# IRVLUTD/GraspTrajOpt

Hardware: AMD Instinct MI355X
Metric: grasp trajectories/sec (higher is better)
Workload: dtype f64

## Files before the change

grasptrajopt_amd/csrc/gto_api.hip:

```cpp
#include <hip/hip_runtime.h>
#include <hipcub/hipcub.hpp>

#include <algorithm>
#include <atomic>
#include <climits>
#include <cmath>
#include <cstdio>
#include <cstdlib>
#include <cstring>
#include <string>
#include <chrono>
#include <memory>
#include <mutex>
#include <thread>
#include <utility>
#include <vector>

#include <sys/prctl.h>

#include "gto_kernels.h"
#include "gto_depth.h"
#include "gto_cloud.h"
#include "gto_retime.h"
#include "gto_observe.h"
// ... 3 lines not shown

#define GTO_VERSION GTO_ABI_VERSION
#ifndef GTO_OBS_DEEP_PD
#define GTO_OBS_DEEP_PD 8
#endif

static std::string g_create_error;

#define GTO_SWEEP_WGS 64

#define GTO_MAX_LANES 8
#define GTO_BASE_PIN_SLOTS 4
#define GTO_STAGE_SLOTS 8
#define GTO_NAP_US 50
#define GTO_NAP_FEW_US 10
#define GTO_OBS_DEEP_MAX 32

struct Tunables {
  int ahead = 8;
  int ahead_few = 4;
  int spec_rej = 4, spec_acc = 4, spec_deep = 32;
  int spec_rej_few = 2, spec_jobs = 20;
  int spec_streak = 4;
  int spec_acc_tail = 2, spec_streak_tail = 2, obs_tg_few_tail = 3;
  int spec_few = 64;
  int obs_deep = 1;
  int dbg_cut = 0;
  int dist_relax = 0;
  int obs_interleave = 2;
  int static_pos = 1;
  int pb_merge = 4;
  int prebroad = 1;
  int seed_pb = 1;
  double pb_min_gain = 0.10;
  int obs_tg = 3;
  int obs_tg_few = 2;
  int obs_tg_wide = 5;
  bool obs_tg_given = false;
  int few_instances = 192;
  int step_nw_few = 8;
  int slots = 512;
  int lanes_max = 1, lane_min = 256, adopt_below = 0;
  int item_hint_forced = 0;
  int item_grid = 1;
  bool debug_timing = false;
  bool lane_debug = false;
};

static void read_tunables(Tunables& t) {
  using F = int Tunables::*;
  struct Row { const char* name; F f, also1, also2; int lo, hi; };
  const int BIG = INT_MAX;
  static const Row rows[] = {
      {"GTO_AHEAD", &Tunables::ahead, &Tunables::ahead_few, nullptr, 1, BIG},
      {"GTO_SPEC_REJ", &Tunables::spec_rej, nullptr, nullptr, 1, GTO_KSPEC},
      {"GTO_SPEC_REJ_FEW", &Tunables::spec_rej_few, nullptr, nullptr, 1, GTO_KSPEC},
      {"GTO_SPEC_STREAK", &Tunables::spec_streak, &Tunables::spec_streak_tail, nullptr, 0, BIG},
      {"GTO_SPEC_STREAK_TAIL", &Tunables::spec_streak_tail, nullptr, nullptr, 0, BIG},
      {"GTO_SPEC_JOBS", &Tunables::spec_jobs, nullptr, nullptr, 1, BIG},
      {"GTO_SPEC_ACC", &Tunables::spec_acc, &Tunables::spec_acc_tail, nullptr, 1, GTO_KSPEC},
      {"GTO_SPEC_ACC_TAIL", &Tunables::spec_acc_tail, nullptr, nullptr, 1, GTO_KSPEC},
      {"GTO_SPEC_DEEP", &Tunables::spec_deep, nullptr, nullptr, 0, BIG},
      {"GTO_SPEC_FEW", &Tunables::spec_few, nullptr, nullptr, 0, BIG},
      {"GTO_OBS_DEEP", &Tunables::obs_deep, nullptr, nullptr, 0, 1},
      {"GTO_PREBROAD", &Tunables::prebroad, nullptr, nullptr, 0, 1},
      {"GTO_SEED_PB", &Tunables::seed_pb, nullptr, nullptr, 0, 1},
      {"GTO_PB_MERGE", &Tunables::pb_merge, nullptr, nullptr, 1, BIG},
      {"GTO_STATIC_POS", &Tunables::static_pos, nullptr, nullptr, 0, 1},
      {"GTO_OBS_INTERLEAVE", &Tunables::obs_interleave, nullptr, nullptr, 0, 2},
      {"GTO_DIST_RELAX", &Tunables::dist_relax, nullptr, nullptr, 0, 1},
      {"GTO_DEBUG_CUT", &Tunables::dbg_cut, nullptr, nullptr, INT_MIN, INT_MAX},
      {"GTO_ITEM_GRID", &Tunables::item_grid, nullptr, nullptr, 0, 1},
      {"GTO_ITEM_HINT", &Tunables::item_hint_forced, nullptr, nullptr, 0, BIG},
      {"GTO_SLOTS", &Tunables::slots, nullptr, nullptr, 1, BIG},
      {"GTO_LANES", &Tunables::lanes_max, nullptr, nullptr, 1, GTO_MAX_LANES},
      {"GTO_LANE_MIN", &Tunables::lane_min, nullptr, nullptr, 1, BIG},
      {"GTO_ADOPT", &Tunables::adopt_below, nullptr, nullptr, 0, BIG},
      {"GTO_OBS_TG", &Tunables::obs_tg, &Tunables::obs_tg_few, &Tunables::obs_tg_few_tail, 1, GTO_MAX_TG},
      {"GTO_OBS_TG_FEW", &Tunables::obs_tg_few, &Tunables::obs_tg_few_tail, nullptr, 1, GTO_MAX_TG},
      {"GTO_OBS_TG_FEW_TAIL", &Tunables::obs_tg_few_tail, nullptr, nullptr, 1, GTO_MAX_TG},
      {"GTO_OBS_TG_WIDE", &Tunables::obs_tg_wide, nullptr, nullptr, 1, GTO_MAX_TG},
      {"GTO_FEW_INSTANCES", &Tunables::few_instances, nullptr, nullptr, INT_MIN, INT_MAX},
  };
  for (const Row& r : rows) {
    const char* e = getenv(r.name);
    if (!e) continue;
    int v = atoi(e);
    v = r.lo == 0 && r.hi == 1 ? (v != 0) : std::max(r.lo, std::min(r.hi, v));
    for (F f : {r.f, r.also1, r.also2})
      if (f) t.*f = v;
  }
  t.obs_tg_given = getenv("GTO_OBS_TG") != nullptr;
  if (const char* e = getenv("GTO_STEP_NW_FEW")) t.step_nw_few = atoi(e) == 8 ? 8 : 4;
  if (const char* e = getenv("GTO_PB_MIN_GAIN")) t.pb_min_gain = atof(e);
  t.debug_timing = getenv("GTO_DEBUG_TIMING") != nullptr;
  t.lane_debug = getenv("GTO_LANE_DEBUG") != nullptr;
  if (t.dbg_cut) fprintf(stderr, "[gto] WARNING: GTO_DEBUG_CUT=%d cuts the obstacle kernel short: timing experiments only, RESULTS ARE GARBAGE\n", t.dbg_cut);
}

using DevBuf = Owned<hipFree>;
using PinBuf = Owned<hipHostFree>;

struct gto_handle {
  int device = 0;
  hipStream_t stream = nullptr;
  bool own_stream = true;
  std::string err;
  gto_solver_opts opts;
  RobotDev rb;
  DevBuf rb_buf, px_buf, py_buf, pz_buf, plink_buf, perm_buf, chunks_buf;
  RobotDev* d_rb = nullptr;
  double *d_px = nullptr, *d_py = nullptr, *d_pz = nullptr;
  int32_t *d_plink = nullptr, *d_perm = nullptr;
  Chunk* d_chunks = nullptr;
  std::vector<PbChunk> pbchunks;
  int pb_C = 0;
  DevBuf d_pbimg;
  std::vector<SceneDev> scenes;
  std::vector<std::vector<DevBuf>> scene_bufs;
  DevBuf scenes_buf;
  SceneDev* d_scenes = nullptr;
  DevBuf state, Qcur, Qtry, vis, screw, blocks, goalblk, ssfixed, ndone, qf, livebuf, qfs, wrecbuf, itembuf, seedmask;
  DevBuf counters;
  unsigned long long last_counters[4] = {0, 0, 0, 0};
  PinBuf h_ndone;
  PinBuf h_progress;
  unsigned long long* d_progress = nullptr;
  unsigned progress_tag = 0;
  Tunables tu;
  int spec_kmax = 1;
  DevBuf dbg;
  std::vector<DevBuf> spare;
  DevBuf in[GTO_STAGE_SLOTS], out[GTO_STAGE_SLOTS];
  PinBuf pin_in[GTO_STAGE_SLOTS], pin_out[GTO_STAGE_SLOTS];
  bool profiling = false;
  std::vector<hipEvent_t> ev;
  std::vector<int> ev_variant;
  std::vector<long long> ev_wgs;
  double last_ms = 0.0;
  int last_launches = 0;
  double prof_ms[GTO_PROF_VARIANTS] = {};
  long long prof_launches[GTO_PROF_VARIANTS] = {}, prof_wgs[GTO_PROF_VARIANTS] = {};
  unsigned long long prof_points[GTO_PROF_VARIANTS] = {};
  size_t lm_lds = 0;
  int np = GTO_NB;
  DevBuf zws;
  hipStream_t lane_stream[GTO_MAX_LANES] = {};
  hipEvent_t lane_event[GTO_MAX_LANES] = {};
  hipStream_t user_lane_stream[GTO_MAX_LANES] = {};
  int n_user_lane_streams = 0;
  double items_per_job_prior = 0.0;
  std::mutex* prof_mu = nullptr;
  DevBuf rt_fac, rt_S, rt_flag, rt_P1, rt_P2, rt_cap, rt_X, rt_T, rt_stat;
  bool rt_fac_ready = false;
  DevBuf ck_xyz, ck_flags, ck_base;
// ... 867 lines not shown
  sp.tol_step = o.tol_step;
  sp.tol_rel_f = o.tol_rel_f;
  sp.lambda0 = o.lambda0;
  sp.dbg_cut = h->tu.dbg_cut;
  sp.interleave = h->tu.obs_interleave == 1;
  sp.static_pos = 0;
  sp.pb_next = 0, sp.pb_tg = 1, sp.pb_ng = 1, sp.pb_pw = 1, sp.pb_verify = 0;
  sp.pb_C = h->pb_C, sp.pb_tab0 = 0, sp.pb_mC = ObsGeom::magic(std::max(1, h->pb_C)), sp.pb_mF = ObsGeom::magic(h->rb.n_frames);
  sp.pb_eps = h->rb.pb_eps;
  sp.pb_npar = h->rb.pb_npar;
  sp.round = sp.parity = 0;
  sp.kcap = h->np == GTO_NB ? GTO_KSPEC : 1;
  sp.k_acc = sp.k_rej = sp.k_eval = 1;
  sp.spec_streak = h->tu.spec_streak;
  return sp;
}

static int ensure_workspace(gto_handle* h, int B) {
  const RobotDev& rb = h->rb;
  const size_t T = h->opts.T, n = rb.n_opt;
  int rc;
  if ((rc = ensure(h, h->state, (size_t)B * sizeof(InstState)))) return rc;
  if ((rc = ensure(h, h->Qcur, (size_t)B * n * T * sizeof(double)))) return rc;
  const size_t kcap = h->np == GTO_NB ? GTO_KSPEC : 1;
  if ((rc = ensure(h, h->Qtry, kcap * B * n * T * sizeof(double)))) return rc;
  const size_t bstride = (size_t)h->np * h->np + h->np + 8;
  if ((rc = ensure(h, h->blocks, (kcap + 1) * B * T * bstride * sizeof(double)))) return rc;
  if ((rc = ensure(h, h->goalblk, (kcap + 1) * B * 2 * bstride * sizeof(double)))) return rc;
  if ((rc = ensure(h, h->ssfixed, (size_t)B * 4 * sizeof(double)))) return rc;
  if ((rc = ensure(h, h->ndone, 64 * GTO_MAX_LANES))) return rc;
  if ((rc = ensure(h, h->qf, (size_t)B * T * rb.n_frames * sizeof(double)))) return rc;
  if ((rc = ensure(h, h->wrecbuf, (size_t)(kcap + 1) * B * T * 8 * sizeof(double)))) return rc;
  if ((rc = ensure(h, h->seedmask, (size_t)B * sizeof(unsigned long long)))) return rc;
  if (!h->h_ndone) HIPCHK(h, pinned_alloc(h->h_ndone, 64));
  if (!h->h_progress) {
    HIPCHK(h, pinned_alloc(h->h_progress, 64 * GTO_MAX_LANES, hipHostMallocMapped));
    std::memset(h->h_progress.get(), 0, 64 * GTO_MAX_LANES);
    HIPCHK(h, hipHostGetDevicePointer((void**)&h->d_progress, h->h_progress.get(), 0));
  }
  return GTO_OK;
}

static BatchPtrs make_ptrs(gto_handle* h, const int32_t* scene_id, const double* qc, const double* goals,
                           const int32_t* n_goals, const double* standoff, const double* base_pos, const double* Q0) {
  BatchPtrs bp = {};
  bp.scene_id = scene_id;
  bp.qc = qc;
  bp.goals = goals;
  bp.n_goals = n_goals;
  bp.standoff = standoff;
  bp.base_pos = base_pos;
  bp.Q0 = Q0;
  bp.state = h->state.as<InstState>();
  bp.Qcur = h->Qcur.as<double>();
  bp.Qtry = h->Qtry.as<double>();
  bp.blocks = h->blocks.as<double>();
  bp.goalblk = h->goalblk.as<double>();
  bp.ss_fixed = h->ssfixed.as<double>();
  bp.n_done = h->ndone.as<int32_t>();
  bp.qf = h->qf.as<double>();
  bp.live = nullptr;
  bp.jobs = nullptr;
  bp.nlive = nullptr;
  bp.next = nullptr;
  bp.qfs = nullptr;
  bp.wrec = h->wrecbuf.as<double>();
// ... 17 lines not shown
    if ((e = hipEventCreate(&ev_)) == hipSuccess) h->ev.push_back(ev_);
  }
  if (e == hipSuccess) {
    if (h->ev_variant.size() <= (size_t)h->last_launches) h->ev_variant.resize(h->last_launches + 1), h->ev_wgs.resize(h->last_launches + 1);
    h->ev_variant[h->last_launches] = variant;
    h->ev_wgs[h->last_launches] = wgs;
    e = hipEventRecord(h->ev[2 * h->last_launches], st);
  }
  if (e != hipSuccess && h->prof_mu) h->prof_mu->unlock();
  HIPCHK(h, e);
  return GTO_OK;
}
static int prof_end(gto_handle* h, hipStream_t st) {
  const hipError_t e = hipEventRecord(h->ev[2 * h->last_launches + 1], st);
  h->last_launches++;
  if (h->prof_mu) h->prof_mu->unlock();
  HIPCHK(h, e);
  return GTO_OK;
}

using InitKernel = decltype(&k_lm_init<GTO_NB>);
static InitKernel lm_init_kernel(int np) { return np == GTO_NB ? k_lm_init<GTO_NB> : k_lm_init<16>; }

struct ObsLaunch {
  int t_begin = 2, nT = 0;
  int fixed_mode = 0;
  bool timed = false;
  bool goal_terms = false;
  int n_jobs = 0;
  int tg = 0;
  bool deep = false;
  bool itemized = false;
  int items_hint = 0;
};
static ObsLaunch init_pass() {
  ObsLaunch o;
  o.t_begin = 0, o.nT = 4, o.fixed_mode = 1;
  return o;
}

static int launch_obstacle(gto_handle* h, hipStream_t st, const BatchPtrs& bp, const SolveParams& sp, int B, const ObsLaunch& o) {
  const int TG = o.fixed_mode ? 1 : std::max(1, std::min(o.tg > 0 ? o.tg : h->tu.obs_tg, o.nT));
  const ObsGeom geo(h->rb.n_cframes, h->rb.n_frames, h->rb.fk_rounds_c, h->rb.n_links, h->rb.n_opt, h->rb.n_chunks, TG, o.nT, h->np);
  const int nG = geo.nG;
  const int nb = o.n_jobs > 0 ? o.n_jobs : B;
  int n_regular = obstacle_grid(nb, nG);
  const bool sweep = o.itemized && o.items_hint > 0 && o.items_hint + GTO_SWEEP_WGS < n_regular && bp.live != nullptr && !o.fixed_mode && !o.deep && h->np == GTO_NB;
  if (sweep) n_regular = 8 * ((o.items_hint + 7) / 8);
  const size_t lds = (size_t)geo.lay.total_doubles * sizeof(double);
  const int n_crew = sweep ? GTO_SWEEP_WGS : 0;
  const dim3 grid(n_regular + n_crew + (o.goal_terms ? 8 * ((nb + 31) / 32) : 0));
  const bool deep_v = h->np == GTO_NB && o.deep;
  if (o.timed) {
    int rc_ = prof_begin(h, st, deep_v ? GTO_PROF_OBSTACLE_FEW : GTO_PROF_OBSTACLE, (long long)grid.x);
    if (rc_) return rc_;
  }
  BatchPtrs bpl = bp;
  if (bpl.work) bpl.work += 64 * (deep_v ? GTO_PROF_OBSTACLE_FEW : GTO_PROF_OBSTACLE);
  const bool listed = bp.live != nullptr && !o.fixed_mode;
  const int32_t* jobs_par = listed ? bp.jobs + (size_t)sp.parity * bp.cap * sp.kcap : nullptr;
  const int32_t* njobs_par = listed ? bp.nlive + GTO_NJOBS(sp.parity) : nullptr;
  const size_t items_cap = (size_t)bp.cap * sp.kcap * (sp.T - 2) + GTO_ITEM_SLACK;
  const int2* items_par = listed && o.itemized ? bp.items + (size_t)sp.parity * items_cap : nullptr;
  const int32_t* nitems_par = listed && o.itemized ? bp.nlive + 8 + sp.parity : nullptr;
  const bool hot = !o.fixed_mode && sp.grad_mode == GTO_GRAD_CENTRAL_DIFF;
  hipLaunchKernelGGL(obstacle_kernel(h->np, o.deep, sweep, hot), grid, dim3(256), lds, st, jobs_par, njobs_par, items_par, nitems_par, geo.nG, geo.m_nG, n_regular, B,
                     h->d_rb, h->d_px, h->d_py, h->d_pz, h->d_chunks, h->d_scenes, bpl, sp, o.t_begin, o.nT, o.fixed_mode, geo, n_crew);
  if (o.timed) return prof_end(h, st);
  return GTO_OK;
}

}

struct LaneCtx {
  hipStream_t st = nullptr;
  BatchPtrs bp;
  SolveParams sp;
  int lo = 0, n = 0, W = 0, cap = 0;
  int room = 0;
  int span_prev = 0;
  int n_resp = 0;
  int k = 0, known_done = 0, seen_round = -1, k_prev = 1;
  int last_plain = -1;
  bool items_ready = false, pb_off = false, handed = false;
  double ratio_max = 0.0;
  long end_us = 0, few_us = 0;
  unsigned long long* h_prog = nullptr;
};

struct Handover { int lane, parity, count, k_prev; };

struct SolveCall {
  gto_handle* h = nullptr;
  int B = 0, L = 1, T = 0, kcap = 1, nF = 0, max_iter = 0;
  int pb_ng = 1;
  bool pb_able = false;
  size_t lane_zws[GTO_MAX_LANES + 1] = {0};
  LaneCtx lanes[GTO_MAX_LANES];
  std::chrono::steady_clock::time_point tp_start;
  std::mutex mu;
  std::vector<Handover> requests;
  int reserved = 0;
  int adopt_limit = 0;
  std::atomic<int> rem0_pub{0}, others_open{0}, failed{0};
};

static int setup_lanes(gto_handle* h, hipStream_t st, SolveParams& sp, BatchPtrs& bp, SolveCall& c) {
  const int B = c.B, T = c.T, kcap = c.kcap, nF = c.nF;
  const int L = c.L = std::max(1, std::min(std::min(h->tu.lanes_max, GTO_MAX_LANES), B / std::max(1, h->tu.lane_min)));
  const int adopt_room = L > 1 ? (L - 1) * std::max(0, h->tu.adopt_below) : 0;
  size_t off_live[GTO_MAX_LANES + 1] = {0}, off_qfs[GTO_MAX_LANES + 1] = {0}, off_items[GTO_MAX_LANES + 1] = {0};
  for (int l = 0; l < L; ++l) {
    LaneCtx& ln = c.lanes[l];
    ln.lo = (int)((long long)B * l / L);
    ln.n = (int)((long long)B * (l + 1) / L) - ln.lo;
    ln.W = std::min(ln.n, h->tu.slots);
    ln.cap = ln.W + (l == 0 ? adopt_room : 0);
// ... 30 lines not shown
    else if (l < h->n_user_lane_streams) ln.st = h->user_lane_stream[l];
    else {
      if (!h->lane_stream[l]) {
        int lo_p = 0, hi_p = 0;
        HIPCHK(h, hipDeviceGetStreamPriorityRange(&lo_p, &hi_p));
        HIPCHK(h, hipStreamCreateWithPriority(&h->lane_stream[l], hipStreamNonBlocking, hi_p));
      }
      ln.st = h->lane_stream[l];
    }
    if (!h->lane_event[l]) HIPCHK(h, hipEventCreateWithFlags(&h->lane_event[l], hipEventDisableTiming));
  }
  HIPCHK(h, hipMemsetAsync(h->ndone.get(), 0, 16 * sizeof(int32_t) * L, st));
  h->progress_tag = h->progress_tag + 1 ? h->progress_tag + 1 : 1;
  for (int l = 0; l < L; ++l) c.lanes[l].bp.progress_tag = (unsigned long long)h->progress_tag << 32;
  if (h->profiling) {
    if ((rc = ensure(h, h->counters, GTO_PROF_VARIANTS * 64 * sizeof(unsigned long long)))) return rc;
    HIPCHK(h, hipMemsetAsync(h->counters.get(), 0, GTO_PROF_VARIANTS * 64 * sizeof(unsigned long long), st));
    bp.work = h->counters.as<unsigned long long>();
    for (int l = 0; l < L; ++l) c.lanes[l].bp.work = bp.work;
  }
  const int pb_tg = std::max(1, std::min(h->tu.obs_tg, T - 2));
  c.pb_ng = (T - 2 + pb_tg - 1) / pb_tg;
  const PbLayout pbl(T, h->rb.n_frames, h->pb_C, h->rb.pb_npar);
  c.pb_able = h->tu.prebroad && h->np == GTO_NB && c.pb_ng <= 64 && h->tu.obs_interleave != 1 && h->rb.n_xst <= GTO_PB_PARK && pbl.pw >= 1 && h->pb_C >= 1;
  for (int l = 0; l < L; ++l) {
    SolveParams& lsp = c.lanes[l].sp;
    lsp.pb_tg = pb_tg, lsp.pb_ng = c.pb_ng, lsp.pb_pw = std::max(1, pbl.pw), lsp.pb_tab0 = pbl.tab0;
    lsp.pb_verify = h->tu.dbg_cut == 10;
  }
  sp.pb_tg = pb_tg, sp.pb_ng = c.pb_ng, sp.pb_pw = std::max(1, pbl.pw), sp.pb_tab0 = pbl.tab0;
  return GTO_OK;
}

static int test_waiting_seeds(gto_handle* h, hipStream_t st, SolveCall& c) {
  if (!c.pb_able || !h->tu.seed_pb) return GTO_OK;
  for (int l = 0; l < c.L; ++l) {
    LaneCtx& ln = c.lanes[l];
    if (ln.n <= ln.W || ln.W <= h->tu.few_instances) continue;
    int rc;
    if (h->profiling && (rc = prof_begin(h, st, GTO_PROF_SEED_TEST, ln.n - ln.W))) return rc;
    hipLaunchKernelGGL(k_seed_broad, dim3(ln.n - ln.W), dim3(256), h->lm_lds, st, h->d_rb, ln.bp, ln.sp, c.B, h->seedmask.as<unsigned long long>());
    if (h->profiling && (rc = prof_end(h, st))) return rc;
    ln.bp.seed_mask = h->seedmask.as<unsigned long long>();
  }
  return GTO_OK;
}

enum StepVariant { STEP_FULL, STEP_FEW, STEP_WIDE };
struct RoundPlan {
  int in_flight = 0;
  int span = 0;
  bool few = false;
  bool interleave = false;
  ObsLaunch obs;
  StepVariant step = STEP_FULL;
  int k_acc = 1, k_rej = 1, spec_streak = 0;
  bool pb_next = false, static_pos = false;
  int k_next = 1;
  bool pb_off = false;
  double ratio_max = 0.0;
};

static RoundPlan plan_round(const gto_handle* h, const SolveCall& c, const LaneCtx& ln) {
  const Tunables& tu = h->tu;
  RoundPlan p;
  p.in_flight = std::min(ln.room, ln.n_resp - ln.known_done);
  p.few = p.in_flight <= tu.few_instances;
  p.span = ln.span_prev ? ln.span_prev : p.in_flight;
  p.interleave = tu.obs_interleave == 1 || (tu.obs_interleave == 2 && p.few);
  p.pb_off = ln.pb_off;
  p.ratio_max = ln.ratio_max;
  p.k_next = ln.k_prev;
  const bool large_call = ln.n_resp > tu.spec_deep;
  ObsLaunch& o = p.obs;
  o.nT = c.T - 2;
  o.timed = h->profiling;
  o.goal_terms = true;
  o.n_jobs = p.span * ln.k_prev;
  o.tg = p.few ? (large_call ? tu.obs_tg_few_tail : tu.obs_tg_few) : tu.obs_tg;
  o.deep = p.few && tu.obs_deep && p.in_flight <= GTO_OBS_DEEP_MAX;
  o.itemized = ln.items_ready && !p.few;
  if (o.itemized && tu.item_grid) {
    const unsigned long long p2 = __atomic_load_n(ln.h_prog + 2, __ATOMIC_RELAXED);
    const int jobs_bound = p.in_flight * ln.k_prev;
    const bool zero_ok = ln.last_plain < ln.seen_round - 1;
    if ((unsigned)(p2 >> 32) == h->progress_tag && ((p2 & 0xfffffull) > 0 || zero_ok) && (p2 & 0xfffffull) < 0xfffffull) {
      const double items_seen = (double)(p2 & 0xfffffull), jobs_seen = (double)((p2 >> 20) & 0xfffull);
      o.items_hint = (int)(1.5 * items_seen) + 256;
      if (jobs_seen > 0 && jobs_seen < 4095) p.ratio_max = std::max(p.ratio_max, items_seen / jobs_seen);
    } else if (h->items_per_job_prior > 0.0) {
      o.items_hint = (int)(1.25 * h->items_per_job_prior * jobs_bound) + 256;
    }
    if (tu.item_hint_forced > 0) o.items_hint = tu.item_hint_forced;
  }
  if (h->np != GTO_NB) {
    p.step = STEP_WIDE;
  } else if (p.few && tu.step_nw_few == 8) {
    p.step = STEP_FEW;
    const int k_budget = std::max(1, tu.spec_jobs / std::max(1, p.in_flight));
    p.k_acc = p.in_flight <= std::min(tu.spec_deep, tu.spec_few) ? std::min(std::min(large_call ? tu.spec_acc_tail : tu.spec_acc, k_budget), h->spec_kmax) : 1;
    p.spec_streak = large_call ? tu.spec_streak_tail : tu.spec_streak;
    p.k_rej = p.in_flight <= tu.spec_few ? std::min(std::max(std::min(tu.spec_rej, k_budget), tu.spec_rej_few), h->spec_kmax) : 1;
    p.k_next = std::max(p.k_acc, p.k_rej);
  } else {
    p.step = STEP_FULL;
    const bool pb_ok = c.pb_able && std::min(ln.W, ln.n) > tu.few_instances;
    if (pb_ok && !p.pb_off && !ln.sp.pb_verify) {
      const unsigned long long p2 = __atomic_load_n(ln.h_prog + 2, __ATOMIC_RELAXED);
      if ((unsigned)(p2 >> 32) == h->progress_tag) {
        const double jobs_seen = (double)((p2 >> 20) & 0xfffull), items_seen = (double)(p2 & 0xfffffull);
        if (jobs_seen > 0 && items_seen > 0 && jobs_seen < 4095 && ln.k >= 12 && items_seen > (1.0 - tu.pb_min_gain) * jobs_seen * c.pb_ng) p.pb_off = true;
      }
    }
    p.pb_next = pb_ok && !p.pb_off && !p.few;
    p.static_pos = tu.static_pos && c.L == 1 && !p.few;
    p.k_next = 1;
  }
  return p;
}
// ... 274 lines not shown
  int n_in_ = 0, n_out_ = 0;
  void* host_[GTO_STAGE_SLOTS] = {};
  size_t bytes_[GTO_STAGE_SLOTS] = {};
};

extern "C" {

int gto_solve_batch_device(gto_handle* h, int32_t B, int32_t n_max, const int32_t* scene_id, const double* qc,
                           const double* goals, const int32_t* n_goals, const double* standoff, const double* base_pos,
                           const double* Q0, double* Q_out, double* dQ_out, double* cost_out, int32_t* iters_out,
                           int32_t* status_out, void* stream) {
  if (!h) return GTO_ERR_INVALID_ARG;
  if (B < 0 || n_max < 1) return fail(h, GTO_ERR_INVALID_ARG, "B must be >= 0 and n_max >= 1");
  if (B == 0) return GTO_OK;
  if (B > GTO_JOB_MASK) return fail(h, GTO_ERR_UNSUPPORTED, "more than 16.7 million instances in one call");
  if (!scene_id || !qc || !goals || !n_goals || !base_pos || !Q0) return fail(h, GTO_ERR_INVALID_ARG, "null input array");
  if (h->scenes.empty()) return fail(h, GTO_ERR_NO_SCENE, "no scene has been set");
  HIPCHK(h, hipSetDevice(h->device));
  hipStream_t st = stream ? (hipStream_t)stream : h->stream;
  int rc = ensure_workspace(h, B);
  if (rc) return rc;
  SolveParams sp = make_params(h, n_max, standoff != nullptr);
  BatchPtrs bp = make_ptrs(h, scene_id, qc, goals, n_goals, standoff, base_pos, Q0);
  h->last_launches = 0;
  h->last_ms = 0.0;
  if (h->dbg) HIPCHK(h, hipMemsetAsync(h->dbg.as<long long>() + 40, 0, 216 * sizeof(long long), st));

  SolveCall c;
  c.h = h, c.B = B, c.T = sp.T, c.kcap = sp.kcap, c.nF = h->rb.n_frames, c.max_iter = sp.max_iter;
  if ((rc = setup_lanes(h, st, sp, bp, c))) return rc;
  const int L = c.L;
  for (int l = 0; l < L; ++l)
    hipLaunchKernelGGL(lm_init_kernel(h->np), dim3(c.lanes[l].n), dim3(256), 0, st, h->d_rb, c.lanes[l].bp, c.lanes[l].sp, B, 0);
  if ((rc = launch_obstacle(h, st, bp, sp, B, init_pass()))) return rc;
  if ((rc = test_waiting_seeds(h, st, c))) return rc;
  if (L > 1) {
    HIPCHK(h, hipEventRecord(h->lane_event[0], st));
    for (int l = 0; l < L; ++l) HIPCHK(h, hipStreamWaitEvent(c.lanes[l].st, h->lane_event[0], 0));
  }
  const int old_slack = prctl(PR_GET_TIMERSLACK);
  if (old_slack > 1000) (void)prctl(PR_SET_TIMERSLACK, 1000UL);
  c.tp_start = std::chrono::steady_clock::now();
  int rc_loop = run_lanes(c);
  {
    double r_ = 0.0;
    for (int l = 0; l < L; ++l) r_ = std::max(r_, c.lanes[l].ratio_max);
    if (r_ > 0.0) h->items_per_job_prior = r_;
  }
  for (int l = 0; l < L && L > 1 && !rc_loop; ++l)
    if (!c.lanes[l].handed) {
      if (hipEventRecord(h->lane_event[l], c.lanes[l].st) != hipSuccess || hipStreamWaitEvent(st, h->lane_event[l], 0) != hipSuccess) {
        h->err = "solve loop: joining the lanes failed";
        rc_loop = GTO_ERR_HIP;
      }
    }
  if (rc_loop)
    for (int l = 0; l < L && L > 1; ++l) (void)hipStreamSynchronize(c.lanes[l].st);
  bp.live = c.lanes[0].bp.live, bp.cap = c.lanes[0].bp.cap;
  if (old_slack > 1000) (void)prctl(PR_SET_TIMERSLACK, (unsigned long)old_slack);
  if (rc_loop) return rc_loop;
  hipLaunchKernelGGL(k_lm_finalize, dim3(B), dim3(64), 0, st, h->d_rb, bp, sp, B, Q_out, dQ_out, cost_out, iters_out, status_out);
  HIPCHK(h, hipGetLastError());
  if (h->dbg && (rc = print_debug_stamps(h, st))) return rc;
  if (h->profiling && (rc = harvest_profile(h, st, bp.work))) return rc;
  return GTO_OK;
}

// ... 455 lines not shown
  int rc = check_scene_ids_host(h, scene_id, B);
  if (rc) return rc;
  HIPCHK(h, hipSetDevice(h->device));
  const size_t ndof = h->rb.ndof, T = h->opts.T;
  std::vector<double> dummy_goal;
  std::vector<int32_t> dummy_n;
  std::vector<double> qc(B * ndof);
  for (int b = 0; b < B; ++b)
    for (size_t i = 0; i < ndof; ++i) qc[b * ndof + i] = Q[((size_t)b * ndof + i) * T];
  if (!with_goals) {
    n_max = 1;
    dummy_goal.assign((size_t)B * 16, 0.0);
    for (int b = 0; b < B; ++b) dummy_goal[b * 16] = dummy_goal[b * 16 + 5] = dummy_goal[b * 16 + 10] = dummy_goal[b * 16 + 15] = 1.0;
    dummy_n.assign(B, 1);
    goals = dummy_goal.data();
    n_goals = dummy_n.data();
    standoff = nullptr;
  }
  Staging io(h);
  const int32_t *d_sid, *d_ng;
  const double *d_qc, *d_goals, *d_so, *d_base, *d_Q0;
  if ((rc = io.in(scene_id, B, &d_sid))) return rc;
  if ((rc = io.in(qc.data(), B * ndof, &d_qc))) return rc;
  if ((rc = io.in(goals, (size_t)B * n_max * 16, &d_goals))) return rc;
  if ((rc = io.in(n_goals, B, &d_ng))) return rc;
  if ((rc = io.in(standoff, (size_t)B * 16, &d_so))) return rc;
  if ((rc = io.in(base_pos, (size_t)B * 3, &d_base))) return rc;
  if ((rc = io.in(Q, B * ndof * T, &d_Q0))) return rc;
  if ((rc = ensure_workspace(h, B))) return rc;
  SolveParams sp = make_params(h, n_max, standoff != nullptr);
  BatchPtrs bp = make_ptrs(h, d_sid, d_qc, d_goals, d_ng, d_so, d_base, d_Q0);
  HIPCHK(h, hipMemsetAsync(bp.n_done, 0, sizeof(int32_t), h->stream));
  hipLaunchKernelGGL(lm_init_kernel(h->np), dim3(B), dim3(256), 0, h->stream, h->d_rb, bp, sp, B, 1 );
  if ((rc = launch_obstacle(h, h->stream, bp, sp, B, init_pass()))) return rc;
  h->last_launches = 0;
  ObsLaunch ev;
  ev.nT = (int)T - 2, ev.timed = h->profiling;
  if ((rc = launch_obstacle(h, h->stream, bp, sp, B, ev))) return rc;
  if (h->profiling) {
    HIPCHK(h, hipStreamSynchronize(h->stream));
    float ms = 0.f;
    HIPCHK(h, hipEventElapsedTime(&ms, h->ev[0], h->ev[1]));
    h->last_ms = ms;
  }
  states.resize(B);
  const size_t bstride = (size_t)h->np * h->np + h->np + 8;
  blocks.resize((size_t)B * T * bstride);
  ssfixed.resize((size_t)B * 4);
  HIPCHK(h, hipMemcpyAsync(states.data(), h->state.get(), B * sizeof(InstState), hipMemcpyDeviceToHost, h->stream));
  HIPCHK(h, hipMemcpyAsync(blocks.data(), h->blocks.as<double>() + (size_t)1 * B * T * bstride,
                           blocks.size() * sizeof(double), hipMemcpyDeviceToHost, h->stream));
  HIPCHK(h, hipMemcpyAsync(ssfixed.data(), h->ssfixed.get(), ssfixed.size() * sizeof(double), hipMemcpyDeviceToHost, h->stream));
  HIPCHK(h, hipStreamSynchronize(h->stream));
  HIPCHK(h, hipGetLastError());
  return GTO_OK;
}

int gto_eval_objective(gto_handle* h, int32_t B, int32_t n_max, const int32_t* scene_id, const double* goals,
                       const int32_t* n_goals, const double* standoff, const double* base_pos, const double* Q,
                       double* f_goal, double* f_obs, double* f_vel, int32_t* goal_argmin) {
  if (!h) return GTO_ERR_INVALID_ARG;
  if (B < 0 || n_max < 1 || !scene_id || !goals || !n_goals || !base_pos || !Q) return fail(h, GTO_ERR_INVALID_ARG, "bad argument");
  if (B == 0) return GTO_OK;
  std::vector<InstState> st;
  std::vector<double> blocks, ssf;
  int rc = eval_common(h, B, n_max, scene_id, goals, n_goals, standoff, base_pos, Q, true, st, blocks, ssf);
  if (rc) return rc;
// ... 1135 lines not shown
```

grasptrajopt_amd/csrc/gto_kernels.h:

```cpp
#pragma once
#include <type_traits>

#include "gto_device.h"

template <int NP>
struct Blk {
  static constexpr int JTJ = 0, JTR = NP * NP, SS = NP * NP + NP, STRIDE = NP * NP + NP + 8;
};
#define BLK_JTJ 0
#define BLK_JTR 64
#define BLK_SS 72
#define BLK_STRIDE 80
#define GTO_MAX_ACTIVE 256
#define GTO_MAX_TG 8
#define GTO_MAX_T 96
#ifndef GTO_LIST_CAP
#define GTO_LIST_CAP 64
#endif

#define GTO_KSPEC 4
#define GTO_JOB_SHIFT 28
#define GTO_JOB_SET_SHIFT 24
#define GTO_JOB_MASK 0x00ffffff
#define GTO_JOB_ENTRY(b, set, cand) ((b) | ((set) << GTO_JOB_SET_SHIFT) | ((cand) << GTO_JOB_SHIFT))
// ... 618 lines not shown
  const int par = sp.parity, NS = sp.kcap + 1;
  if (!SWEEP && listed && bid == 0 && tid == 0) {
    bp.nlive[GTO_NLIVE(1 - par)] = bp.nlive[GTO_NJOBS(1 - par)] = 0;
    bp.nlive[8 + 1 - par] = 0;
  }
  if (is_goal) {
    if (gi_ >= n_act || le < 0) return;
    const int bg = le & GTO_JOB_MASK, gcand = le >> GTO_JOB_SHIFT;
    if (bp.state[bg].done || (listed && bp.state[bg].first)) return;
    double* s_fr2 = smem_obs + wave * GTO_GOAL_SCRATCH(NP);
    double* s_q2 = s_fr2 + 2 * GTO_MAX_FRAMES * 12;
    double* s_ga = s_q2 + 2 * GTO_MAX_DOF;
    double* s_gs = s_ga + 48;
#ifdef GTO_DEBUG_LONGEST_WG
    const bool dbg_goal = bp.dbg && bg == 0 && gcand == 0 && lane == 0;
    if (dbg_goal) bp.dbg[31] = clock64();
#endif
    trial_goal_terms_wave<NP>(rb, bp, sp, B, bg, lane, listed ? GTO_JOB_SET(le) : (bp.state[bg].slot + 1 + gcand) % NS, gcand, bp.state + bg, s_q2, s_fr2, s_ga, s_gs);
#ifdef GTO_DEBUG_LONGEST_WG
    if (dbg_goal) bp.dbg[32] = clock64();
#endif
    return;
  }
  for (;;) {
  {
  const int t0v = t_begin + grp_id * TG;
  const bool static_only = fixed_mode && t0v >= 2;
  const int t0w = static_only ? 0 : t0v;
  const bool inter = sp.interleave && !fixed_mode;
  const int wstep = inter ? nG : 1, w0 = inter ? t_begin + grp_id : t0w;
  const int ng = static_only ? 1 : (inter ? geo.q_nT + (grp_id < geo.r_nT ? 1 : 0) : min(TG, (fixed_mode ? 2 : t_begin + nT) - t0v));
  auto wp = [&](int kq_) { return w0 + kq_ * wstep; };
  if (sp.dbg_cut == 5 && (le >= 0 || bi < 0)) goto next_item;

  const int bic = min(bi, (listed ? bp.cap * sp.kcap : B) - 1);
  const int Fq = geo.Fq;
  const double* __restrict__ qfp = listed ? bp.qfs + ((((size_t)par * bp.cap * sp.kcap + bic) * T) + w0) * Fq : bp.qf + ((size_t)bic * T + w0) * Fq;
  const int qstride = wstep * Fq;
  const int tq = fast_div(tid, F, geo.m_F);
  const int fo_t = tid < ng * F ? rb->cf_orig[tid - tq * F] : -1;
  const int jtv = tid < ng * F ? rb->cf_type[tid - tq * F] : GTO_JOINT_FIXED;
  const double qfv = fo_t >= 0 ? qfp[fo_t + tq * qstride] : 0.0;
  const int nt = geo.nt;
  double tabv[6];
#pragma unroll
  for (int u = 0; u < 6; ++u) tabv[u] = tid + 256 * u < nt ? rb->fk_tab_c[tid + 256 * u] : 0.0;
  if ((itemized ? rbid : bi) >= n_act || le < 0) goto next_item;
  const int b = le & GTO_JOB_MASK, cand = le >> GTO_JOB_SHIFT;
  const bool sparse = listed;
  const InstState* st = bp.state + b;
  const bool dbg_wg = bp.dbg && b == 0 && grp_id == nG - 1;
#ifdef GTO_DEBUG_LONGEST_WG
  const long long t_wg0 = bp.dbg ? clock64() : 0;
#endif
  if (dbg_wg && tid == 0) bp.dbg[10] = clock64();
  if (sp.dbg_cut == 6) goto next_item;
  if (!listed && st->done) goto next_item;
  const int set_out = listed ? GTO_JOB_SET(le) : (st->slot + 1 + cand) % NS;
  const int C = geo.C;
  double ssfix = 0.0;
  if (!fixed_mode && tid < ng) ssfix = bp.ss_fixed[4 * b + (wp(tid) < sp.ts ? 2 : 3)];
#pragma unroll
  for (int u = 0; u < 6; ++u)
    if (tid + 256 * u < nt) s_ktab[tid + 256 * u] = tabv[u];
  for (int k = tid + 256 * 6; k < nt; k += 256) s_ktab[k] = rb->fk_tab_c[k];
  if (sp.dbg_cut == 7) goto next_item;
// ... 1040 lines not shown
  const int* s_flag = reinterpret_cast<const int*>(s_tab);
  const double ss_a = s_tab[38], ss_o = s_tab[39];
  double* __restrict__ wr = bp.wrec + (((size_t)set_n * B + b) * T + 2) * 8;
  for (int i = tid; i < m * 8; i += NT) {
    const int sI = i >> 3;
    if (!s_flag[sI / TG]) wr[i] = (i & 7) == 0 ? 0.0 + (sI + 2 < sp.ts ? ss_a : ss_o) : 0.0;
  }
}
__device__ __forceinline__ void pb_list_groups(const BatchPtrs& bp, const SolveParams& sp, int par_n, int entry, int pos, bool hit, int lane) {
  const bool on = lane < sp.pb_ng && (hit || sp.pb_verify);
  const unsigned long long mask = __ballot(on);
  int base = 0;
  if (lane == 0 && mask) base = atomicAdd(bp.nlive + 8 + par_n, __popcll(mask));
  base = __shfl(base, 0, 64);
  if (on) bp.items[(size_t)par_n * ((size_t)bp.cap * sp.kcap * (sp.T - 2) + GTO_ITEM_SLACK) + base + __popcll(mask & ((1ull << lane) - 1ull))] =
              make_int2(entry, (pos << 8) | lane | (hit ? 0 : 0x80));
}

template <int NT>
__device__ __forceinline__ void prebroad_tail(const RobotDev* __restrict__ rb,
                                              const BatchPtrs& bp, const SolveParams& sp, int B, int b, int scene_b, int set_n, int pos_next,
                                              const double* __restrict__ s_qt, double* __restrict__ smem, int tid) {
  const bool dbg_t = bp.dbg && b == 0 && tid == 0;
  pb_test<NT>(rb, bp, sp, b, scene_b, s_qt, smem, tid, true);
  if (dbg_t) bp.dbg[38] = clock64();
  pb_settle_records<NT>(bp, sp, B, b, set_n, smem, tid);
  if (tid < 64) {
    const int* s_flag = reinterpret_cast<const int*>(smem + sp.pb_tab0);
    pb_list_groups(bp, sp, 1 - sp.parity, GTO_JOB_ENTRY(b, set_n, 0), pos_next, tid < sp.pb_ng && s_flag[tid] != 0, tid);
  }
  if (dbg_t) bp.dbg[39] = clock64();
}

__global__ __launch_bounds__(256) void k_seed_broad(const RobotDev* __restrict__ rb, BatchPtrs bp, SolveParams sp, int B, unsigned long long* __restrict__ mask_out) {
  constexpr int NT = 256;
  const int b = bp.b0 + bp.w0 + blockIdx.x, tid = threadIdx.x;
  if (b >= bp.n_total) return;
  extern __shared__ __attribute__((aligned(16))) double smem[];
  __shared__ int s_bad;
  const int T = sp.T, m = T - 2, n = rb->n_opt, F = rb->n_frames;
  double* __restrict__ s_qt = smem + 80 * (size_t)m;
  const int scene_b = bp.scene_id[b];
  if (tid == 0) s_bad = 0;
  __syncthreads();
  {
    const double* __restrict__ qf0 = bp.qf + (size_t)b * T * F;
    bool bad = false;
    for (int i = tid; i < T * F; i += NT) bad |= !(fabs(qf0[i]) < INFINITY);
    if (bad) s_bad = 1;
    const double* __restrict__ Qt = bp.Qtry + (size_t)b * n * T;
    for (int i = tid; i < m * 8; i += NT) s_qt[i] = (i & 7) < n ? Qt[(size_t)(i & 7) * T + (i >> 3) + 2] : 0.0;
  }
  __syncthreads();
  if (s_bad) {
    if (tid == 0) mask_out[b] = ~0ull;
    return;
  }
  pb_test<NT>(rb, bp, sp, b, scene_b, s_qt, smem, tid, false);
  pb_settle_records<NT>(bp, sp, B, b, 1, smem, tid);
  if (tid < 64) {
    const int* s_flag = reinterpret_cast<const int*>(smem + sp.pb_tab0);
    const unsigned long long mk = __ballot(tid < sp.pb_ng && s_flag[tid] != 0);
    if (tid == 0) mask_out[b] = mk;
  }
}

template <int NP>
__global__ __launch_bounds__(256) void k_lm_init(const RobotDev* __restrict__ rb, BatchPtrs bp, SolveParams sp, int B, int raw) {
  const int b = blockIdx.x + bp.b0, tid = threadIdx.x, bl = blockIdx.x;
  __shared__ double s_gaff[48];
  __shared__ double s_gscr[2 * NP * 6];
  __shared__ double s_q[2 * GTO_MAX_DOF];
  __shared__ double s_fr[2 * GTO_MAX_FRAMES * 12];
  const int T = sp.T, n = rb->n_opt;
  InstState* st = bp.state + b;
  if (tid == 0) {
    st->f = INFINITY;
    st->lambda = sp.lambda0;
    st->nu = 2.0;
    st->pred[0] = 0.0;
    st->ncand = 1;
    st->cflags = 0;
    st->nz0 = st->nz1 = 0ull;
    st->slot = 0;
    st->first = 1;
    st->done = 0;
    st->status = GTO_STATUS_MAX_ITER;
    st->evals = 0;
    st->argmin_cur = 0;
  }
  if (bp.live && tid == 0) {
    if (bl < bp.w0) bp.live[bl] = b, bp.jobs[bl] = GTO_JOB_ENTRY(b, 1, 0);
    if (bl == 0) {
      *bp.next = bp.b0 + bp.w0;
      bp.nlive[GTO_NLIVE(0)] = bp.nlive[GTO_NJOBS(0)] = bp.w0;
      bp.nlive[GTO_NLIVE(1)] = bp.nlive[GTO_NJOBS(1)] = 0;
      bp.nlive[8] = bp.nlive[9] = 0;
    }
  }
  const double* Q0b = bp.Q0 + (size_t)b * rb->ndof * T;
  double* Qt = bp.Qtry + (size_t)b * n * T;
  double* Qc = bp.Qcur + (size_t)b * n * T;
  for (int idx = tid; idx < n * T; idx += 256) {
    const int j = idx / T, t = idx % T;
    double v = Q0b[(size_t)rb->opt_index[j] * T + t];
    if (!raw) {
      if (t < 2) v = bp.qc[(size_t)b * rb->ndof + rb->opt_index[j]];
      else v = v < rb->lower[j] ? rb->lower[j] : (v > rb->upper[j] ? rb->upper[j] : v);
    }
    Qt[idx] = v;
    Qc[idx] = v;
  }
  __syncthreads();
  {
    const int F = rb->n_frames;
    double* qf = bp.qf + (size_t)b * T * F;
    for (int idx = tid; idx < T * F; idx += 256) {
      const int t = idx / F, i = idx - t * F, dq = rb->q_index[i];
      double v = 0.0;
      if (dq >= 0) {
        const int j = rb->opt_of_dof[dq];
        v = j >= 0 ? Qt[(size_t)j * T + t] : Q0b[(size_t)dq * T + t];
      }
      qf[idx] = v;
      if (bp.live && bl < bp.w0) bp.qfs[(size_t)bl * T * F + idx] = v;
    }
  }
  if (tid < 64) trial_goal_terms_wave<NP>(rb, bp, sp, B, b, tid, 1, 0, st, s_q, s_fr, s_gaff, s_gscr);
}

__device__ __forceinline__ double fast_rcp(double x) {
  double r = __builtin_amdgcn_rcp(x);
  r = fma(fma(-x, r, 1.0), r, r);
  r = fma(fma(-x, r, 1.0), r, r);
  return r;
}

template <int J>
__device__ __forceinline__ double bcast_col8(double v) {
  constexpr int q = J & 3, QP = q | (q << 2) | (q << 4) | (q << 6);
  constexpr int BM = (J >> 2) ? 0x5 : 0xA;
  int lo = __builtin_amdgcn_update_dpp(0, __double2loint(v), QP, 0xf, 0xf, false);
  int hi = __builtin_amdgcn_update_dpp(0, __double2hiint(v), QP, 0xf, 0xf, false);
  lo = __builtin_amdgcn_update_dpp(lo, lo, 0x141, 0xf, BM, false);
  hi = __builtin_amdgcn_update_dpp(hi, hi, 0x141, 0xf, BM, false);
  return __hiloint2double(hi, lo);
}
template <int J>
__device__ __forceinline__ void gj_pivot8(double& S, int& bad, int r, int c) {
  const double pjj = __hiloint2double(__builtin_amdgcn_readlane(__double2hiint(S), J * 9),
                                      __builtin_amdgcn_readlane(__double2loint(S), J * 9));
  const double prj = bcast_col8<J>(S);
  const double pjc = __shfl(S, J * 8 + c, 64);
  if (!(pjj > 0.0)) bad = 1;
  const double piv = fast_rcp(pjj);
  const double tcol = -prj * piv;
  const double in_row = (c == J) ? piv : pjc * piv;
  const double off_row = (c == J) ? tcol : fma(tcol, pjc, S);
  S = (r == J) ? in_row : off_row;
}
__device__ __forceinline__ int gj_invert8(double& S, int r, int c, int n = 8) {
// ... 2443 lines not shown
```

Measured before the change: 570,400.

## Deduplicate identical instances in init obstacle pass and seed-broadphase all slots

Adds a kernel that, within each 64-instance wave group, finds instances whose scene, base pose and first two timesteps of joint frames match their predecessor, and maps each to a representative head. The fixed-mode init obstacle pass skips non-head instances, and a spread kernel copies the head's fixed terms to the duplicates. It also runs the seed broadphase test on the in-slot instances so their group lists are prepared up front, and ignores progress hints from those seeded rounds. This avoids redundant collision work when batches contain repeated starts, at the cost of extra launches and reliance on exact bitwise equality.

```diff
diff --git a/grasptrajopt_amd/csrc/gto_api.hip b/grasptrajopt_amd/csrc/gto_api.hip
--- a/grasptrajopt_amd/csrc/gto_api.hip
+++ b/grasptrajopt_amd/csrc/gto_api.hip
@@ -59,6 +59,8 @@
   int pb_merge = 4;
   int prebroad = 1;
   int seed_pb = 1;
+  int seed_pb_all = 1;
+  int init_dedup = 1, init_dedup_min = 1280;
   double pb_min_gain = 0.10;
   int obs_tg = 3;
   int obs_tg_few = 2;
@@ -92,6 +94,9 @@
       {"GTO_OBS_DEEP", &Tunables::obs_deep, nullptr, nullptr, 0, 1},
       {"GTO_PREBROAD", &Tunables::prebroad, nullptr, nullptr, 0, 1},
       {"GTO_SEED_PB", &Tunables::seed_pb, nullptr, nullptr, 0, 1},
+      {"GTO_SEED_PB_ALL", &Tunables::seed_pb_all, nullptr, nullptr, 0, 1},
+      {"GTO_INIT_DEDUP", &Tunables::init_dedup, nullptr, nullptr, 0, 1},
+      {"GTO_INIT_DEDUP_MIN", &Tunables::init_dedup_min, nullptr, nullptr, 0, BIG},
       {"GTO_PB_MERGE", &Tunables::pb_merge, nullptr, nullptr, 1, BIG},
       {"GTO_STATIC_POS", &Tunables::static_pos, nullptr, nullptr, 0, 1},
       {"GTO_OBS_INTERLEAVE", &Tunables::obs_interleave, nullptr, nullptr, 0, 2},
@@ -147,7 +152,7 @@
   std::vector<std::vector<DevBuf>> scene_bufs;
   DevBuf scenes_buf;
   SceneDev* d_scenes = nullptr;
-  DevBuf state, Qcur, Qtry, vis, screw, blocks, goalblk, ssfixed, ndone, qf, livebuf, qfs, wrecbuf, itembuf, seedmask;
+  DevBuf state, Qcur, Qtry, vis, screw, blocks, goalblk, ssfixed, ndone, qf, livebuf, qfs, wrecbuf, itembuf, seedmask, inithead;
   DevBuf counters;
   unsigned long long last_counters[4] = {0, 0, 0, 0};
   PinBuf h_ndone;
@@ -1081,6 +1086,7 @@
   if ((rc = ensure(h, h->qf, (size_t)B * T * rb.n_frames * sizeof(double)))) return rc;
   if ((rc = ensure(h, h->wrecbuf, (size_t)(kcap + 1) * B * T * 8 * sizeof(double)))) return rc;
   if ((rc = ensure(h, h->seedmask, (size_t)B * sizeof(unsigned long long)))) return rc;
+  if ((rc = ensure(h, h->inithead, (size_t)B * sizeof(int32_t)))) return rc;
   if (!h->h_ndone) HIPCHK(h, pinned_alloc(h->h_ndone, 64));
   if (!h->h_progress) {
     HIPCHK(h, pinned_alloc(h->h_progress, 64 * GTO_MAX_LANES, hipHostMallocMapped));
@@ -1164,10 +1170,11 @@
   bool deep = false;
   bool itemized = false;
   int items_hint = 0;
+  const int32_t* rep = nullptr;
 };
-static ObsLaunch init_pass() {
+static ObsLaunch init_pass(const int32_t* rep = nullptr) {
   ObsLaunch o;
-  o.t_begin = 0, o.nT = 4, o.fixed_mode = 1;
+  o.t_begin = 0, o.nT = 4, o.fixed_mode = 1, o.rep = rep;
   return o;
 }
 
@@ -1194,7 +1201,7 @@
   const int32_t* njobs_par = listed ? bp.nlive + GTO_NJOBS(sp.parity) : nullptr;
   const size_t items_cap = (size_t)bp.cap * sp.kcap * (sp.T - 2) + GTO_ITEM_SLACK;
   const int2* items_par = listed && o.itemized ? bp.items + (size_t)sp.parity * items_cap : nullptr;
-  const int32_t* nitems_par = listed && o.itemized ? bp.nlive + 8 + sp.parity : nullptr;
+  const int32_t* nitems_par = listed && o.itemized ? bp.nlive + 8 + sp.parity : (o.fixed_mode ? o.rep : nullptr);
   const bool hot = !o.fixed_mode && sp.grad_mode == GTO_GRAD_CENTRAL_DIFF;
   hipLaunchKernelGGL(obstacle_kernel(h->np, o.deep, sweep, hot), grid, dim3(256), lds, st, jobs_par, njobs_par, items_par, nitems_par, geo.nG, geo.m_nG, n_regular, B,
                      h->d_rb, h->d_px, h->d_py, h->d_pz, h->d_chunks, h->d_scenes, bpl, sp, o.t_begin, o.nT, o.fixed_mode, geo, n_crew);
@@ -1215,6 +1222,7 @@
   int k = 0, known_done = 0, seen_round = -1, k_prev = 1;
   int last_plain = -1;
   bool items_ready = false, pb_off = false, handed = false;
+  bool seed_round0 = false;
   double ratio_max = 0.0;
   long end_us = 0, few_us = 0;
   unsigned long long* h_prog = nullptr;
@@ -1311,6 +1319,16 @@
   return GTO_OK;
 }
 
+static int run_init_pass(gto_handle* h, hipStream_t st, const BatchPtrs& bp, const SolveParams& sp, int B) {
+  if (!h->tu.init_dedup || 4 * (long long)B <= h->tu.init_dedup_min) return launch_obstacle(h, st, bp, sp, B, init_pass());
+  int32_t* rep = h->inithead.as<int32_t>();
+  hipLaunchKernelGGL(k_init_heads, dim3((B + 255) / 256), dim3(256), 0, st, h->d_rb, bp, sp.T, B, rep);
+  const int rc = launch_obstacle(h, st, bp, sp, B, init_pass(rep));
+  if (rc) return rc;
+  hipLaunchKernelGGL(k_ss_fixed_spread, dim3((B + 255) / 256), dim3(256), 0, st, bp, B, rep);
+  return GTO_OK;
+}
+
 static int test_waiting_seeds(gto_handle* h, hipStream_t st, SolveCall& c) {
   if (!c.pb_able || !h->tu.seed_pb) return GTO_OK;
   for (int l = 0; l < c.L; ++l) {
@@ -1318,9 +1336,13 @@
     if (ln.n <= ln.W || ln.W <= h->tu.few_instances) continue;
     int rc;
     if (h->profiling && (rc = prof_begin(h, st, GTO_PROF_SEED_TEST, ln.n - ln.W))) return rc;
-    hipLaunchKernelGGL(k_seed_broad, dim3(ln.n - ln.W), dim3(256), h->lm_lds, st, h->d_rb, ln.bp, ln.sp, c.B, h->seedmask.as<unsigned long long>());
+    hipLaunchKernelGGL(k_seed_broad, dim3(ln.n - ln.W), dim3(256), h->lm_lds, st, h->d_rb, ln.bp, ln.sp, c.B, h->seedmask.as<unsigned long long>(), 0);
     if (h->profiling && (rc = prof_end(h, st))) return rc;
     ln.bp.seed_mask = h->seedmask.as<unsigned long long>();
+    if (h->tu.seed_pb_all) {
+      hipLaunchKernelGGL(k_seed_broad, dim3(ln.W), dim3(256), h->lm_lds, st, h->d_rb, ln.bp, ln.sp, c.B, h->seedmask.as<unsigned long long>(), 1);
+      ln.items_ready = ln.seed_round0 = true;
+    }
   }
   return GTO_OK;
 }
@@ -1363,7 +1385,8 @@
     const unsigned long long p2 = __atomic_load_n(ln.h_prog + 2, __ATOMIC_RELAXED);
     const int jobs_bound = p.in_flight * ln.k_prev;
     const bool zero_ok = ln.last_plain < ln.seen_round - 1;
-    if ((unsigned)(p2 >> 32) == h->progress_tag && ((p2 & 0xfffffull) > 0 || zero_ok) && (p2 & 0xfffffull) < 0xfffffull) {
+    const bool of_seeds = ln.seed_round0 && ln.seen_round < 2;
+    if ((unsigned)(p2 >> 32) == h->progress_tag && ((p2 & 0xfffffull) > 0 || zero_ok) && !of_seeds && (p2 & 0xfffffull) < 0xfffffull) {
       const double items_seen = (double)(p2 & 0xfffffull), jobs_seen = (double)((p2 >> 20) & 0xfffull);
       o.items_hint = (int)(1.5 * items_seen) + 256;
       if (jobs_seen > 0 && jobs_seen < 4095) p.ratio_max = std::max(p.ratio_max, items_seen / jobs_seen);
@@ -1704,7 +1727,7 @@
   const int L = c.L;
   for (int l = 0; l < L; ++l)
     hipLaunchKernelGGL(lm_init_kernel(h->np), dim3(c.lanes[l].n), dim3(256), 0, st, h->d_rb, c.lanes[l].bp, c.lanes[l].sp, B, 0);
-  if ((rc = launch_obstacle(h, st, bp, sp, B, init_pass()))) return rc;
+  if ((rc = run_init_pass(h, st, bp, sp, B))) return rc;
   if ((rc = test_waiting_seeds(h, st, c))) return rc;
   if (L > 1) {
     HIPCHK(h, hipEventRecord(h->lane_event[0], st));
@@ -2226,7 +2249,7 @@
   BatchPtrs bp = make_ptrs(h, d_sid, d_qc, d_goals, d_ng, d_so, d_base, d_Q0);
   HIPCHK(h, hipMemsetAsync(bp.n_done, 0, sizeof(int32_t), h->stream));
   hipLaunchKernelGGL(lm_init_kernel(h->np), dim3(B), dim3(256), 0, h->stream, h->d_rb, bp, sp, B, 1 );
-  if ((rc = launch_obstacle(h, h->stream, bp, sp, B, init_pass()))) return rc;
+  if ((rc = run_init_pass(h, h->stream, bp, sp, B))) return rc;
   h->last_launches = 0;
   ObsLaunch ev;
   ev.nT = (int)T - 2, ev.timed = h->profiling;
diff --git a/grasptrajopt_amd/csrc/gto_kernels.h b/grasptrajopt_amd/csrc/gto_kernels.h
--- a/grasptrajopt_amd/csrc/gto_kernels.h
+++ b/grasptrajopt_amd/csrc/gto_kernels.h
@@ -674,6 +674,9 @@
   const int ng = static_only ? 1 : (inter ? geo.q_nT + (grp_id < geo.r_nT ? 1 : 0) : min(TG, (fixed_mode ? 2 : t_begin + nT) - t0v));
   auto wp = [&](int kq_) { return w0 + kq_ * wstep; };
   if (sp.dbg_cut == 5 && (le >= 0 || bi < 0)) goto next_item;
+  if constexpr (!HOT && !SWEEP && PD == GTO_OBS_MAIN_PD) {
+    if (fixed_mode && nitems_par != nullptr && bi < B && nitems_par[bi] != bi) goto next_item;
+  }
 
   const int bic = min(bi, (listed ? bp.cap * sp.kcap : B) - 1);
   const int Fq = geo.Fq;
@@ -1780,10 +1783,11 @@
   if (dbg_t) bp.dbg[39] = clock64();
 }
 
-__global__ __launch_bounds__(256) void k_seed_broad(const RobotDev* __restrict__ rb, BatchPtrs bp, SolveParams sp, int B, unsigned long long* __restrict__ mask_out) {
+__global__ __launch_bounds__(256) void k_seed_broad(const RobotDev* __restrict__ rb, BatchPtrs bp, SolveParams sp, int B, unsigned long long* __restrict__ mask_out, int in_slots) {
   constexpr int NT = 256;
-  const int b = bp.b0 + bp.w0 + blockIdx.x, tid = threadIdx.x;
-  if (b >= bp.n_total) return;
+  const int bl = in_slots ? (int)blockIdx.x : bp.w0 + (int)blockIdx.x;
+  const int b = bp.b0 + bl, tid = threadIdx.x;
+  if (b >= bp.n_total || (in_slots && bl >= bp.w0)) return;
   extern __shared__ __attribute__((aligned(16))) double smem[];
   __shared__ int s_bad;
   const int T = sp.T, m = T - 2, n = rb->n_opt, F = rb->n_frames;
@@ -1802,14 +1806,17 @@
   __syncthreads();
   if (s_bad) {
     if (tid == 0) mask_out[b] = ~0ull;
+    if (in_slots && tid < 64) pb_list_groups(bp, sp, 0, GTO_JOB_ENTRY(b, 1, 0), bl, tid < sp.pb_ng, tid);
     return;
   }
   pb_test<NT>(rb, bp, sp, b, scene_b, s_qt, smem, tid, false);
   pb_settle_records<NT>(bp, sp, B, b, 1, smem, tid);
   if (tid < 64) {
     const int* s_flag = reinterpret_cast<const int*>(smem + sp.pb_tab0);
-    const unsigned long long mk = __ballot(tid < sp.pb_ng && s_flag[tid] != 0);
+    const bool hit = tid < sp.pb_ng && s_flag[tid] != 0;
+    const unsigned long long mk = __ballot(hit);
     if (tid == 0) mask_out[b] = mk;
+    if (in_slots) pb_list_groups(bp, sp, 0, GTO_JOB_ENTRY(b, 1, 0), bl, hit, tid);
   }
 }
 
@@ -1875,6 +1882,34 @@
     }
   }
   if (tid < 64) trial_goal_terms_wave<NP>(rb, bp, sp, B, b, tid, 1, 0, st, s_q, s_fr, s_gaff, s_gscr);
+}
+
+#define GTO_HEAD_BLOCK 64
+__global__ __launch_bounds__(256) void k_init_heads(const RobotDev* __restrict__ rb, BatchPtrs bp, int T, int B, int32_t* __restrict__ rep) {
+  static_assert(GTO_HEAD_BLOCK == 64, "one ballot per block");
+  const int b = blockIdx.x * 256 + threadIdx.x, lane = threadIdx.x & (GTO_HEAD_BLOCK - 1);
+  bool head = true;
+  if (b < B && lane != 0) {
+    unsigned long long diff = (unsigned long long)(unsigned)(bp.scene_id[b] ^ bp.scene_id[b - 1]);
+    const unsigned long long* __restrict__ bs = reinterpret_cast<const unsigned long long*>(bp.base_pos) + (size_t)b * 3;
+    for (int i = 0; i < 3; ++i) diff |= bs[i] ^ bs[i - 3];
+    const int F = rb->n_frames, stride = T * F;
+    const unsigned long long* __restrict__ q = reinterpret_cast<const unsigned long long*>(bp.qf) + (size_t)b * stride;
+    for (int i = 0; i < 2 * F; ++i) diff |= q[i] ^ q[i - stride];
+    head = diff != 0ull;
+  }
+  const unsigned long long heads = __ballot(head);
+  if (b < B) rep[b] = b - lane + 63 - __clzll(heads & (~0ull >> (63 - lane)));
+}
+__global__ __launch_bounds__(256) void k_ss_fixed_spread(BatchPtrs bp, int B, const int32_t* __restrict__ rep) {
+  const int b = blockIdx.x * 256 + threadIdx.x;
+  if (b >= B) return;
+  const int r = rep[b];
+  if (r == b) return;
+  const double2* __restrict__ src = reinterpret_cast<const double2*>(bp.ss_fixed + 4 * (size_t)r);
+  double2* __restrict__ dst = reinterpret_cast<double2*>(bp.ss_fixed + 4 * (size_t)b);
+  const double2 v0 = src[0], v1 = src[1];
+  dst[0] = v0, dst[1] = v1;
 }
 
 __device__ __forceinline__ double fast_rcp(double x) {
```

New measurement: 595,200, median of 6. 1.04x the previous value.
